# alexfreudenberg/miraculix

Hardware: AMD Instinct MI355X
Metric: effective GFLOP/s for dgemm_compressed (2-bit SNP x fp64) (higher is better)
Workload: dtype f64; 1 GPU; 1000000x50000 (SNPs x indiv), ncol=32, dgemm_compressed N+T per step, uncentred; snps=1000000, indiv=50000, ncol=32, parallelism=snp-shard1, form=one process per GPU

## Files before the change

miraculix_amd/csrc/mxa_api.cpp:

```cpp
#include "../../include/miraculix_amd.h"
#include "mxa_internal.h"

#include <algorithm>
#include <atomic>
#include <chrono>
#include <cstdarg>
#include <cstdio>
#include <cstdlib>
#include <cstring>
#include <mutex>
#include <string>
#include <vector>

namespace mxa {

static int g_err = 0;
static char g_errmsg[512] = "";

Options &options() { static Options o; return o; }
Profile &profile() { static Profile p; return p; }
Geometry &last_geometry() { static Geometry g; return g; }
static bool g_profile_on = true;
static std::atomic<int> g_engine{[] {
  const char *e = getenv("MXA_ENGINE");
// ... 585 lines not shown
  const PackedMatrix *G_tn_single = no_plain ? &gemm_operand(h, trans, true) : nullptr;
  const bool small_ok = (engine == 0 || (engine == 4 && n <= 2)) && k >= 128;
  auto guarded_small = [&](int c0, int nc, const PackedMatrix *G_tn, hipEvent_t e0, hipEvent_t e1, int *splits_out, const int **flag_ptr) -> int {
    I8Chain ch; ch.S0 = kSmallS0[nc]; ch.S1 = kSmallS1[nc];
    const bool fb_lut = nc <= 2 && !no_plain;
    GemmPlan pf = fb_lut ? plan_lut(m, G.k_pad, nc) : plan_gemm(m, G.k_pad, nc);
    bool fast_fb = nc >= 2;
    if (fast_fb) {
      const size_t one = (size_t)pf.n_pad * pf.m_pad, need = one * pf.splits;
      fast_fb = partial_budget(w, need, one) >= need;
    }
    ch.fp64_rows = !fast_fb;
    const int r0 = gemm_i8_reserve(G, nc, ch.S0, G_tn, w, s);
    if (r0) return r0;
    if (ch.S1) {
      const int r1 = gemm_i8_reserve(G, nc, ch.S1, G_tn, w, s);
      if (r1 == 1) return 1;
      if (r1 == 2) ch.S1 = 0;
    }
    const double *dBc = dB + (size_t)c0 * ldb;
    double *dCc = dC + (size_t)c0 * ldc;
    const int *d_flag = nullptr;
    for (int cls = 0; cls < (ch.S1 ? 2 : 1); cls++) {
      ch.my_class = cls; ch.first = cls == 0;
      const int rc = gemm_i8_device(G, trans, nc, dBc, ldb, dCc, ldc, fill_rows, centered, d_sumB + c0, d_sumfB + c0, h->d_f, w, s, cls == 0 ? e0 : nullptr, cls == 0 ? e1 : nullptr,
                                    cls == 0 ? splits_out : nullptr, 2, &d_flag, w.d_colpart, 0, G_tn, nullptr, &ch);
      if (rc != 3) return 1;
    }
    if (fast_fb) {
      if (ensure_partials(w, pf, s)) return 1;
      if (fb_lut) { if (launch_lut(G, dBc, ldb, nc, w.d_P, pf, s, d_flag)) return 1; }
      else {
        const bool trf = gemm_use_tr(pf, h, trans);
        if (launch_pack_B(dBc, ldb, k, nc, w.d_Bp, G.k_pad, pf.n_pad, pf.c, s, nullptr, 0, -1, d_flag)) return 1;
        if (launch_gemm(gemm_operand(h, trans, trf), w.d_Bp, w.d_P, pf, 0, s, next_ctr(w), 0, -1, d_flag, trf)) return 1;
      }
      if (launch_finish(w.d_P, pf, m, nc, dCc, ldc, fill_rows, trans ? 1 : 0, centered, d_sumB + c0, d_sumfB + c0, h->d_f, s, nullptr, 0, 0, d_flag, nullptr)) return 1;
    }
    if (flag_ptr) *flag_ptr = d_flag;
    return 0;
  };
  if (small_ok && n <= kSmallNMaxColsHost) {
    const char *e_tn = getenv("MXA_I8_TN");
    const bool tn_ab = e_tn && atoi(e_tn) != 0;
    const PackedMatrix *G_tn = no_plain ? G_tn_single : (tn_ab && n <= 2 && !h->single) ? &gemm_operand(h, trans, true) : nullptr;
    int splits8 = 1;
    const int *d_flag = nullptr;
    const int rcx = guarded_small(0, n, G_tn, pe0, pe1, &splits8, &d_flag);
    if (rcx == 1) return 1;
    if (rcx == 0) {
      std::lock_guard<std::mutex> lk(g_prof_mutex);
      Geometry &geo = last_geometry();
      geo.m = m; geo.k = k; geo.n = n; geo.splits = splits8; geo.a = 0; geo.c = 0; geo.path = 4; geo.d_flag = d_flag; geo.flag_dev = h->device;
      h->prof_pending[slot] = prof;
      return 0;
    }
  }
  if (centered && launch_colsums(dB, ldb, k, n, trans ? nullptr : h->d_f, w.d_colpart, d_sumB, d_sumfB, s)) return 1;
  auto i8_engine_product = [&](int S, double *stats_base, hipEvent_t e0, hipEvent_t e1, int *splits_out) -> int {
    const int rc = gemm_i8_device(G, trans, n, dB, ldb, dC, ldc, fill_rows, centered, d_sumB, d_sumfB, h->d_f, w, s, e0, e1, splits_out, 0, nullptr, nullptr, S, G_tn_single, stats_base);
    if (rc != 2 || !G_tn_single) return rc;
    const int cmax = (6 * 32) / (S > 0 ? S : 7);
    if (cmax < 1) return 2;
    const int chunks = (n + cmax - 1) / cmax, per = (n + chunks - 1) / chunks;
    if (chunks < 2) return 2;
    for (int c0 = 0; c0 < n; c0 += per) {
      const int nc = std::min(per, n - c0);
      const int rcc = gemm_i8_device(G, trans, nc, dB + (size_t)c0 * ldb, ldb, dC + (size_t)c0 * ldc, ldc, fill_rows, centered, d_sumB + c0, d_sumfB + c0, h->d_f, w, s,
// ... 42 lines not shown
  const bool use_lut = n <= 2 && !no_plain;
  GemmPlan p = use_lut ? plan_lut(m, G.k_pad, n) : plan_gemm(m, G.k_pad, n);
  int splits_per_group = p.splits;
  if (!use_lut) {
    const size_t one = (size_t)p.n_pad * p.m_pad, need = one * p.splits;
    const size_t budget = partial_budget(w, need, one);
    if (budget < need) {
      splits_per_group = (int)std::max<size_t>(1, budget / one);
      GemmPlan pg = p; pg.splits = splits_per_group;
      if (ensure_partials(w, pg, s)) return 1;
    }
  }
  if (splits_per_group == p.splits && ensure_partials(w, p, s)) return 1;
  clock_mark("partials");
  {
    std::lock_guard<std::mutex> lk(g_prof_mutex);
    Geometry &geo = last_geometry();
    geo.m = m; geo.k = k; geo.n = n; geo.splits = p.splits; geo.a = p.a; geo.c = p.c; geo.path = use_lut ? 1 : 0;
  }
  const bool tr = !use_lut && gemm_use_tr(p, h, trans);
  const PackedMatrix &GL = gemm_operand(h, trans, tr);
  int mode = gemm_default_mode(p.c);
  const int *d_E = nullptr;
  if (!use_lut && (mode == 2 || mode == 3)) {
    if (w.cap_exp < (size_t)n) {
      MXA_HIP(hipStreamSynchronize(s));
      if (w.d_exp) { MXA_HIP(hipFree(w.d_exp)); w.d_exp = nullptr; w.cap_exp = 0; }
      MXA_HIP(hipMalloc(reinterpret_cast<void **>(&w.d_exp), sizeof(int) * (size_t)n));
      w.cap_exp = n;
    }
    if (launch_colexp(dB, ldb, k, n, w.d_colpart, w.d_exp, 0, s, w.d_denflag, kDenMaxSpan, -100000)) return 1;
    d_E = w.d_exp;
  }
  if (!use_lut && launch_pack_B(dB, ldb, k, n, w.d_Bp, G.k_pad, p.n_pad, p.c, s, d_E, 0, -1, nullptr, mode == 3 && !tr)) return 1;
  if (prof) MXA_HIP(hipEventRecord(pe0, s));
  if (splits_per_group < p.splits) {
    const size_t stride = (size_t)p.n_pad * p.m_pad;
    for (int pass = 0; pass < (d_E ? 2 : 1); pass++) {
      const int *gate = pass ? w.d_denflag : nullptr;
      if (pass && launch_pack_B(dB, ldb, k, n, w.d_Bp, G.k_pad, p.n_pad, p.c, s, nullptr, 0, -1, gate)) return 1;
      for (int sb = 0; sb < p.splits; sb += splits_per_group) {
        const int se = std::min(p.splits, sb + splits_per_group);
        if ((size_t)(se - sb) * stride > w.cap_P) { set_error(4, "internal: a group of %d K splits exceeds the partial-sum workspace", se - sb); return 1; }
        if (launch_gemm(GL, w.d_Bp, w.d_P, p, pass ? 0 : mode, s, next_ctr(w), sb, se, gate, tr, sb)) return 1;
        const int group = (sb > 0 ? 1 : 0) | (se < p.splits ? 2 : 0);
        if (launch_finish(w.d_P, p, m, n, dC, ldc, fill_rows, trans ? 1 : 0, centered, d_sumB, d_sumfB, h->d_f, s, pass ? nullptr : d_E, 0, 0, gate, nullptr, se - sb, group)) return 1;
      }
      if (!pass && prof) { MXA_HIP(hipEventRecord(pe1, s)); h->prof_pending[slot] = true; }
    }
    return 0;
  }
  int rc = use_lut ? launch_lut(G, dB, ldb, n, w.d_P, p, s) : launch_gemm(GL, w.d_Bp, w.d_P, p, mode, s, next_ctr(w), 0, -1, nullptr, tr);
  if (prof && !rc) { MXA_HIP(hipEventRecord(pe1, s)); h->prof_pending[slot] = true; }
  if (!rc && d_E) {
    rc = launch_pack_B(dB, ldb, k, n, w.d_Bp, G.k_pad, p.n_pad, p.c, s, nullptr, 0, -1, w.d_denflag);
    if (!rc) rc = launch_gemm(GL, w.d_Bp, w.d_P, p, 0, s, next_ctr(w), 0, -1, w.d_denflag, tr);
  }
  if (!rc) rc = launch_finish(w.d_P, p, m, n, dC, ldc, fill_rows, trans ? 1 : 0, centered, d_sumB, d_sumfB, h->d_f, s, d_E, 0, 0, nullptr, d_E ? w.d_denflag : nullptr);
  return rc;
}


constexpr int kPipeChunks = 8;
static const size_t kPipeMinBytes = (size_t)32 << 20;

static int pipe_setup(Handle *h) {
  for (hipStream_t &ps : h->pipe) if (!ps) MXA_HIP(hipStreamCreateWithFlags(&ps, hipStreamNonBlocking));
  for (hipEvent_t &e : h->pev) if (!e) MXA_HIP(hipEventCreateWithFlags(&e, hipEventDisableTiming));
  return 0;
}

static int gemm_host_pipelined(Handle *h, bool trans, int n, const double *B, long ldb, bool b_host, bool b_local, double *C, long ldc, bool c_host, bool c_local,
                               long fill_rows) {
  const int engine = g_engine.load();
  if ((engine != 0 && engine != 3) || n < 3 || getenv("MXA_DIAG")) return 2;
  if (engine == 0 && n <= kSmallNMaxColsHost) return 2;
  const PackedMatrix &G = trans ? h->snp_major : h->ind_major;
  const long m = G.rows, k = G.k;
  const size_t b_bytes = b_host ? sizeof(double) * (size_t)k * n : 0, c_bytes = c_host ? sizeof(double) * (size_t)m * n : 0;
  if (std::max(b_bytes, c_bytes) < kPipeMinBytes) return 2;
  const bool kmode = b_bytes >= c_bytes;
  const bool centered = options().centered;
  if (centered && !h->has_f) { set_error(6, "dgemm_compressed: centring requested but no allele frequencies were supplied to plink2compressed"); return 1; }
  if (n > h->max_n) h->max_n = n;
  if (ensure_workspace(h, n) || pipe_setup(h)) return 1;
  harvest_profile(h);
  Workspace &w = h->ws;
  hipStream_t s = h->stream;
  if (grow(&w.d_colpart, &w.cap_colpart, (size_t)n * (128 * (kPipeChunks + 1) + 2) + 16)) return 1;
// ... 765 lines not shown
```

miraculix_amd/csrc/mxa_internal.h:

```cpp
#pragma once
#include <hip/hip_runtime.h>
#include <cstddef>
#include <cstdint>
#include <functional>
#include <utility>
#include <vector>
#include "mxa_plan.h"

namespace mxa {

constexpr int kWaves = 4;
constexpr int kKStep = 16;
constexpr int kSlabSteps = 8;
constexpr int kSlabK = kKStep * kSlabSteps;
constexpr int kSlabBytes = kSlabK / 4;
constexpr int kRowAlign = 512;
constexpr int kTileRows = 256;
constexpr int kTileBytes = kTileRows * kSlabBytes;

constexpr long kMaxBlocksPerLaunch = 1L << 23;
template <typename Launch>
inline void launch_in_block_chunks(long blocks, Launch &&launch) {
  for (long b0 = 0; b0 < blocks; b0 += kMaxBlocksPerLaunch) launch((unsigned)(blocks - b0 < kMaxBlocksPerLaunch ? blocks - b0 : kMaxBlocksPerLaunch), b0);
}
// ... 106 lines not shown
int bed_range_to_handle(const char *base, long snps_total, long indiv, long snp_begin, long snp_end, int max_n, int device, void **out,
                        double *f_out_local);
constexpr int kMaxShards = 64;
struct PartList { const double *p[kMaxShards]; int count; };
int launch_reduce_parts(const PartList &parts, long m, int n, double *dC, long ldc, long fill_rows, hipStream_t s);

void set_error(int code, const char *fmt, ...);
void clear_error();
bool check_hip(hipError_t e, const char *func, int line);
#define MXA_HIP(x) do { if (!::mxa::check_hip((x), __func__, __LINE__)) return 1; } while (0)
void debug_info(const char *fmt, ...);
struct CallClock {
  bool on = false;
  double t0 = 0.0, last = 0.0;
  char line[512]; int len = 0;
  static double now();
  void start(bool enabled) { on = enabled; len = 0; line[0] = 0; if (on) t0 = last = now(); }
  void mark(const char *what);
  void report(const char *head);
};
extern thread_local CallClock *tl_call_clock;
inline void clock_mark(const char *what) { if (tl_call_clock && tl_call_clock->on) tl_call_clock->mark(what); }

int launch_recode(const uint8_t *d_src, size_t src_pitch, long row0, long nrows, long k, long k_bit_offset,
                  PackedMatrix &dst, hipStream_t s);
constexpr int kDenUp = 900;
constexpr int kDenMaxSpan = 800;
constexpr int kI8ExactMaxDigits = 24;
int launch_colspan(const double *dB, long ldb, long k, int n, double *d_part, int *d_out3, hipStream_t s);
int launch_colexp_from_part(const double *d_part, int n, int *d_E, int bias, hipStream_t s);
int launch_colexp(const double *dB, long ldb, long k, int n, double *d_part, int *d_E, int bias, hipStream_t s, int *d_flag = nullptr, int max_span = 0,
                  int min_emax = 0, bool reset_flag = true);
int launch_pack_B(const double *dB, long ldb, long k, int n, double *dBp, long k_pad, int n_pad, int c, hipStream_t s, const int *d_E = nullptr, long S0 = 0,
                  long S_cnt = -1, const int *run_if_set = nullptr, bool rowscale = false);
int launch_colsums(const double *dB, long ldb, long k, int n, const double *d_f , double *d_part,
                   double *d_sumB, double *d_sumfB, hipStream_t s);
GemmPlan plan_gemm(long m, long k_pad, int n, const GemmPlan *ksplits_like = nullptr);
int gemm_default_mode(int c);
int launch_gemm(const PackedMatrix &G, const double *dBp, double *dP, const GemmPlan &p, int mode, hipStream_t s, int *d_ctr, int split_begin = 0, int split_end = -1,
                const int *run_if_set = nullptr, bool tr = false, int p_split0 = 0);
GemmPlan plan_lut(long m, long k_pad, int n);
int launch_lut(const PackedMatrix &G, const double *dB, long ldb, int n, double *dP, const GemmPlan &p, hipStream_t s, const int *run_if_set = nullptr);
int launch_finish(const double *dP, const GemmPlan &p, long m, int n, double *dC, long ldc, long fill_rows, int mode_trans,
                  bool centered, const double *d_sumB, const double *d_sumfB, const double *d_f, hipStream_t s, const int *d_E = nullptr, int e_splits = 0,
                  int e_stride = 0, const int *run_if_set = nullptr, const int *unscaled_if_set = nullptr, int group_splits = 0, int group = 0);
int ensure_dyn_lds(const void *func, int bytes, unsigned long long *mask);
int launch_transpose_2bit(const uint8_t *d_in, long rows, long cols, uint8_t *d_out, hipStream_t s);
int launch_allele_freq(const uint8_t *d_plink, long snps, long indiv, double *d_f, hipStream_t s);
int launch_plink_lut(uint8_t *d, size_t nbytes, hipStream_t s);
int launch_sparse_times_plink(const uint8_t *dP, size_t pitch, long entries, int nIdx, const int *d_rowIdx, const int *d_colIdx, const double *d_val,
                              double *dC_slab, long ldc, long e_base, long e_count, hipStream_t s);
struct I8Chain { int S0 = 0, S1 = 0, my_class = 0; bool first = true; bool fp64_rows = true; };
int gemm_i8_device(const PackedMatrix &G, bool trans, int n, const double *dB, long ldb, double *dC, long ldc, long fill_rows, bool centered, double *d_sumB,
                   double *d_sumfB, const double *d_f, Workspace &w, hipStream_t s, hipEvent_t ev0, hipEvent_t ev1, int *splits_out, int guard = 0,
                   const int **flag_out = nullptr, double *colsum_scratch = nullptr, int S_override = 0, const PackedMatrix *G_tn = nullptr,
                   double *stats_part = nullptr, const I8Chain *chain = nullptr);
int gemm_i8_reserve(const PackedMatrix &G, int n, int S, const PackedMatrix *G_tn, Workspace &w, hipStream_t s);

int ld_window_any(const char *who, const unsigned char *plink, long snps, long indiv, long window, const int *last, double *out, long ldb, bool scores, int flag,
                  bool is_plink, const double *freq);
int ld_pairwise_any(const char *who, const unsigned char *plink, long snps, long indiv, long window, const int *last, double *out, long ldb, bool scores, int flag);

int launch_dgemm(bool ta, bool tb, long M, long N, long K, double alpha, const double *A, long lda, const double *B, long ldb, double beta, double *C, long ldc,
                 bool lower_only, hipStream_t s);
int launch_potrf_inv_block(double *A, long ld, int nb, long offset, int *info, double *inv_out, hipStream_t s);

}
```

miraculix_amd/csrc/mxa_kernels.hip:

```cpp
#include "mxa_internal.h"
#include "mxa_queue.h"
#include <algorithm>
#include <cstdio>
#include <cstdlib>
#include <vector>

namespace mxa {


__device__ __forceinline__ uint32_t recode16(uint32_t w) {
  const uint32_t H = (w >> 1) & 0x55555555u, L = w & 0x55555555u;
  return ((H & L) << 1) | (H & ~L);
}

__global__ void __launch_bounds__(256) k_recode(const uint8_t *__restrict__ src, size_t src_pitch, long src_row_bytes,
                                                long nrows, long k, uint8_t *__restrict__ dst, long dst_row0, long nslabs, long rows_blocks, long blk0) {
  const long bid = blk0 + blockIdx.x;
  const long rblk = bid % rows_blocks, sgrp = bid / rows_blocks;
  const int rr = threadIdx.x >> 3, part = threadIdx.x & 7;
  const long r = rblk * 32 + rr;
  const long slab = sgrp * 4 + (part >> 1);
  if (r >= nrows || slab >= nslabs) return;
  const long b = slab * kSlabBytes + (part & 1) * 16;
  uint32_t w[4] = {0u, 0u, 0u, 0u};
  const uint8_t *p = src + (size_t)r * src_pitch + b;
  if (b + 16 <= src_row_bytes && (reinterpret_cast<size_t>(p) & 3) == 0) {
    const uint32_t *q = reinterpret_cast<const uint32_t *>(p);
    w[0] = q[0]; w[1] = q[1]; w[2] = q[2]; w[3] = q[3];
  } else {
    for (int u = 0; u < 16; u++)
      if (b + u < src_row_bytes) w[u >> 2] |= (uint32_t)p[u] << (8 * (u & 3));
  }
#pragma unroll
  for (int i = 0; i < 4; i++) {
    uint32_t x = recode16(w[i]);
    const long valid = k - 4 * (b + 4 * i);
    if (valid <= 0) x = 0;
    else if (valid < 16) x &= (1u << (2 * valid)) - 1u;
    w[i] = x;
  }
  const long R = dst_row0 + r;
  const size_t off = ((size_t)(R / kTileRows) * nslabs + (size_t)slab) * kTileBytes + (size_t)(R % kTileRows) * kSlabBytes + (part & 1) * 16;
  *reinterpret_cast<uint4 *>(dst + off) = make_uint4(w[0], w[1], w[2], w[3]);
}

int launch_recode(const uint8_t *d_src, size_t src_pitch, long row0, long nrows, long k, long ,
                  PackedMatrix &dst, hipStream_t s) {
  if (nrows <= 0) return 0;
  const long rows_blocks = (nrows + 31) / 32, slab_groups = (dst.nslabs + 3) / 4;
  const long grid = rows_blocks * slab_groups;
  for (long b0 = 0; b0 < grid; b0 += kMaxBlocksPerLaunch) {
    const long nb = std::min(kMaxBlocksPerLaunch, grid - b0);
    hipLaunchKernelGGL(k_recode, dim3((unsigned)nb), dim3(256), 0, s, d_src, src_pitch, (k + 3) / 4, nrows, k, dst.d, row0, dst.nslabs, rows_blocks, b0);
  }
  MXA_HIP(hipGetLastError());
  return 0;
}

__host__ __device__ __forceinline__ long gemm_k_index(long S, int kk) { return (S >> 3) * 128 + 16 * (kk & 7) + 8 * (kk >> 3) + (S & 7); }

__global__ void __launch_bounds__(256) k_pack_B(const double *__restrict__ B, long ldb, long k, int n,
                                                double *__restrict__ Bp, long total, int C, long S_total, const int *__restrict__ E, int up, long S0, long S_cnt,
                                                const int *__restrict__ run_if_set, int rowscale) {
  if (run_if_set && *run_if_set == 0) return;
  for (long idx = (long)blockIdx.x * blockDim.x + threadIdx.x; idx < total; idx += (long)gridDim.x * blockDim.x) {
    const int l = (int)(idx & 63);
    const long sh = idx >> 6;
    const int h = (int)(sh % C);
    const long cs = sh / C;
    const long S = S0 + cs % S_cnt;
    const int chunk = (int)(cs / S_cnt);
    const long row = gemm_k_index(S, l >> 2);
    const int col = chunk * 4 * C + 4 * h + (l & 3);
    double v = 0.0;
    if (row < k && col < n) {
      v = B[row + (long)col * ldb];
      if (E) v = ldexp(v, up - E[col] - (rowscale ? 2 * (int)(row & 15) : 0));
    }
    Bp[(((size_t)chunk * S_total + S) * C + h) * 64 + l] = v;
  }
}

__global__ void __launch_bounds__(256) k_colmax_partial(const double *__restrict__ B, long ldb, long k, double *__restrict__ part, int n, int want_min) {
  const int j = blockIdx.y, c = blockIdx.x;
  const long per = (k + 63) / 64;
  const long c0 = c * per, c1 = std::min<long>(k, c0 + per);
  const double inf = __longlong_as_double(0x7ff0000000000000ll);
  double m = 0.0, lo = inf;
  for (long r = c0 + threadIdx.x; r < c1; r += 256) {
    const double a = fabs(B[r + (long)j * ldb]);
    m = (a <= 1.7976931348623157e308) ? fmax(m, a) : inf;
    if (a > 0.0) lo = fmin(lo, a);
  }
  __shared__ double sh[256], sl[256];
  sh[threadIdx.x] = m; sl[threadIdx.x] = lo;
  __syncthreads();
// ... 41 lines not shown
  __shared__ int s_span[256], s_emax[256], s_bad[256];
  int span = 0, emin_max = 1 << 20, bad = 0;
  for (int j = threadIdx.x; j < n; j += 256) {
    double m = 0.0;
    for (int c = 0; c < 64; c++) m = fmax(m, part[(size_t)j * 64 + c]);
    if (!isfinite(m)) { bad = 1; continue; }
    if (m > 0.0) {
      double lo = m;
      for (int c = 0; c < 64; c++) lo = fmin(lo, part[((size_t)n + j) * 64 + c]);
      int e = 0, el = 0;
      (void)frexp(m, &e); (void)frexp(lo, &el);
      span = max(span, e - el); emin_max = min(emin_max, e);
    }
  }
  s_span[threadIdx.x] = span; s_emax[threadIdx.x] = emin_max; s_bad[threadIdx.x] = bad;
  __syncthreads();
  for (int w = 128; w > 0; w >>= 1) {
    if ((int)threadIdx.x < w) {
      s_span[threadIdx.x] = max(s_span[threadIdx.x], s_span[threadIdx.x + w]); s_emax[threadIdx.x] = min(s_emax[threadIdx.x], s_emax[threadIdx.x + w]);
      s_bad[threadIdx.x] |= s_bad[threadIdx.x + w];
    }
    __syncthreads();
  }
  if (threadIdx.x == 0) { out[0] = s_span[0]; out[1] = s_emax[0] == (1 << 20) ? 0 : s_emax[0]; out[2] = s_bad[0]; }
}
int launch_colspan(const double *dB, long ldb, long k, int n, double *d_part, int *d_out3, hipStream_t s) {
  hipLaunchKernelGGL(k_colmax_partial, dim3(64, n), dim3(256), 0, s, dB, ldb, k, d_part, n, 1);
  hipLaunchKernelGGL(k_colspan_final, dim3(1), dim3(256), 0, s, d_part, n, d_out3);
  MXA_HIP(hipGetLastError());
  return 0;
}

int launch_pack_B(const double *dB, long ldb, long k, int n, double *dBp, long k_pad, int n_pad, int c, hipStream_t s, const int *d_E, long S0, long S_cnt,
                  const int *run_if_set, bool rowscale) {
  const long S_total = k_pad / 16;
  if (S_cnt < 0) S_cnt = S_total - S0;
  const long total = S_cnt * (long)(n_pad / 4) * 64;
  if (total <= 0) return 0;
  const int grid = (int)std::min<long>((total + 255) / 256, 256L * 64);
  hipLaunchKernelGGL(k_pack_B, dim3(grid), dim3(256), 0, s, dB, ldb, k, n, dBp, total, c, S_total, d_E, kDenUp, S0, S_cnt, run_if_set, rowscale ? 1 : 0);
  MXA_HIP(hipGetLastError());
  return 0;
}

constexpr int kColChunks = 64;

__global__ void __launch_bounds__(256) k_colsum_partial(const double *__restrict__ B, long ldb, long k,
                                                        const double *__restrict__ f, double *__restrict__ part) {
  const int j = blockIdx.y, c = blockIdx.x;
  const long per = (k + kColChunks - 1) / kColChunks;
  const long c0 = c * per, c1 = std::min<long>(k, c0 + per);
  double s1 = 0.0, s2 = 0.0;
  for (long r = c0 + threadIdx.x; r < c1; r += 256) {
    const double b = B[r + (long)j * ldb];
    s1 += b;
    if (f) s2 = fma(f[r], b, s2);
  }
  __shared__ double sh1[256], sh2[256];
  sh1[threadIdx.x] = s1; sh2[threadIdx.x] = s2;
  __syncthreads();
  for (int w = 128; w > 0; w >>= 1) {
    if ((int)threadIdx.x < w) { sh1[threadIdx.x] += sh1[threadIdx.x + w]; sh2[threadIdx.x] += sh2[threadIdx.x + w]; }
    __syncthreads();
  }
  if (threadIdx.x == 0) {
    part[((size_t)j * kColChunks + c) * 2 + 0] = sh1[0];
    part[((size_t)j * kColChunks + c) * 2 + 1] = sh2[0];
  }
}

__global__ void k_colsum_final(const double *__restrict__ part, int n, double *__restrict__ sumB, double *__restrict__ sumfB) {
  const int j = blockIdx.x * blockDim.x + threadIdx.x;
  if (j >= n) return;
// ... 260 lines not shown
              Pbase[(size_t)col * Cfg::kRowsWG + row] = out;
            }
          }
        }
      }
      asm volatile("s_waitcnt lgkmcnt(0)" ::: "memory");
      __builtin_amdgcn_wave_barrier();
    }
    if (DIAG && threadIdx.x == 0 && diag) {
      diag[2 * (size_t)bid] = t1 - t0; diag[2 * (size_t)bid + 1] = r1 - r0;
      diag[2 * (size_t)nunits + 2 * (size_t)bid] = rt_begin; diag[2 * (size_t)nunits + 2 * (size_t)bid + 1] = r0;
      diag[4 * (size_t)nunits + bid] = __builtin_amdgcn_s_memrealtime();
    }
    if (next < 0) break;
    u = un; bid = next;
    asm volatile("s_waitcnt vmcnt(0)" ::: "memory");
    __syncthreads();
  }
}

int gemm_default_mode(int) {
  return 3;
}

static long device_cus() {
  static const long r = [] {
    int dev = 0; hipDeviceProp_t prop;
    if (hipGetDevice(&dev) != hipSuccess || hipGetDeviceProperties(&prop, dev) != hipSuccess) { (void)hipGetLastError(); return 256L; }
    return (long)prop.multiProcessorCount;
  }();
  return r > 0 ? r : 256;
}

GemmPlan plan_gemm(long m, long k_pad, int n, const GemmPlan *ksplits_like) { return plan_gemm_host(m, k_pad, n, device_cus(), ksplits_like); }

template <int A, int C, int MODE, bool TR = false>
static int launch_gemm_t(const PackedMatrix &G, const double *dBp, double *dP, const GemmPlan &p, hipStream_t s, int split_begin, int split_end, const int *run_if_set,
                         int *d_ctr, int p_split0) {
  using Cfg = GemmCfg<A, C>;
  static unsigned long long attr_mask = 0;
  if (ensure_dyn_lds(reinterpret_cast<const void *>(&k_gemm<A, C, MODE, false, TR>), Cfg::kLds, &attr_mask)) return 1;
  const long nunits = (long)p.rowblocks * p.nchunks * (split_end - split_begin);
  if (nunits > 0x3fffffffL) { set_error(3, "launch too large"); return 1; }
  if (nunits <= 0) return 0;
  if (!d_ctr) { set_error(4, "internal: k_gemm needs its queue counters"); return 1; }
  static int per_cu[64] = {};
  int dev = 0;
  MXA_HIP(hipGetDevice(&dev));
  if (!per_cu[dev & 63]) {
    int nb = 0;
    MXA_HIP(hipOccupancyMaxActiveBlocksPerMultiprocessor(&nb, reinterpret_cast<const void *>(&k_gemm<A, C, MODE, false, TR>), 256, Cfg::kLds));
    hipDeviceProp_t prop;
    MXA_HIP(hipGetDeviceProperties(&prop, dev));
    per_cu[dev & 63] = std::max(1, std::min(nb, gemm_wg_per_cu(C))) * prop.multiProcessorCount;
  }
  const long grid = std::min<long>(nunits, per_cu[dev & 63]);
  constexpr int xcd_order = 1;
  const KSplit ks{p.s1, p.l1, p.r1, p.l2};
  const int long_groups = (std::min(split_end, p.s1) - std::min(split_begin, p.s1)) * p.nchunks;
  const int g8 = xcd_order ? (long_groups & ~7) : 0;
  MXA_HIP(hipMemsetAsync(d_ctr, 0, 9 * sizeof(int), s));
  static const bool diag_on = getenv("MXA_DIAG") != nullptr;
  if (!TR && diag_on && ((A == 8 && C == 8) || (A == 16 && C == 1)) && split_begin == 0 && split_end == p.splits && !run_if_set) {
    static unsigned long long attr2 = 0;
    if (ensure_dyn_lds(reinterpret_cast<const void *>(&k_gemm<A, C, MODE, true>), Cfg::kLds, &attr2)) return 1;
    unsigned long long *d_diag = nullptr;
    MXA_HIP(hipMalloc(reinterpret_cast<void **>(&d_diag), sizeof(unsigned long long) * 5 * nunits));
    MXA_HIP(hipMemsetAsync(d_diag, 0, sizeof(unsigned long long) * 5 * nunits, s));
    hipLaunchKernelGGL((k_gemm<A, C, MODE, true>), dim3((unsigned)grid), dim3(256), Cfg::kLds, s, G.d, G.pitch, dBp, p.n_pad / 4, dP,
                       p.m_pad, p.n_pad, p.rowblocks, p.nchunks, p.slabs_total, ks, xcd_order, d_diag, split_begin, (const int *)nullptr, (int)nunits, d_ctr, g8, p_split0);
    MXA_HIP(hipStreamSynchronize(s));
    std::vector<unsigned long long> h(5 * nunits);
    MXA_HIP(hipMemcpy(h.data(), d_diag, sizeof(unsigned long long) * 5 * nunits, hipMemcpyDeviceToHost));
    std::vector<double> ghz, cyc;
    for (long i = 0; i < nunits; i++) if (h[2 * i + 1]) {
      const int sp = (int)(i < (long)g8 * p.rowblocks ? ((i & 7) + 8 * ((i >> 3) / p.rowblocks)) / p.nchunks : (i / p.rowblocks) / p.nchunks);
      const int len = ksplit_len(ks, sp);
      ghz.push_back((double)h[2 * i] / (double)h[2 * i + 1] * 0.1); cyc.push_back((double)h[2 * i] / len);
    }
    std::sort(ghz.begin(), ghz.end()); std::sort(cyc.begin(), cyc.end());
    if (!ghz.empty()) printf("MXA_DIAG k_gemm<%d,%d,%d>: %ld pieces on %ld workgroups (splits %d = %d x %d + short x %d), in-kernel clock median %.3f GHz (min %.3f max %.3f); shader cycles per slab median %.0f (ideal %d)\n",
                             A, C, MODE, nunits, grid, p.splits, p.s1, p.l1, p.l2, ghz[ghz.size() / 2], ghz.front(), ghz.back(), cyc[cyc.size() / 2], kSlabSteps * A * C * 16 * 2);
    double ticks = 0.0;
    for (long i = 0; i < nunits; i++) ticks += (double)h[2 * i + 1];
    printf("MXA_DIAG k_gemm: K loops of all pieces = %.3f ms if packed perfectly on %ld resident slots (compare with the kernel duration)\n", ticks * 1e-5 / (double)grid, grid);
    {
      double life = 0; unsigned long long first = ~0ull, last = 0;
      for (long i = 0; i < nunits; i++) {
        const unsigned long long b = h[2 * nunits + 2 * i], e = h[4 * nunits + i];
        life += (double)(e - b);
        first = std::min(first, b); last = std::max(last, e);
      }
      printf("MXA_DIAG k_gemm: mean piece lifetime %.1f us; span first begin -> last end %.3f ms; sum of lifetimes / slots = %.3f ms\n",
             life / nunits * 1e-2, (double)(last - first) * 1e-5, life * 1e-5 / (double)grid);
      std::vector<std::pair<unsigned long long, int>> ev;
      ev.reserve(2 * nunits);
      for (long i = 0; i < nunits; i++) { ev.emplace_back(h[2 * nunits + 2 * i], +1); ev.emplace_back(h[4 * nunits + i], -1); }
      std::sort(ev.begin(), ev.end());
      const unsigned long long win = 200000;
      double idle[3] = {0, 0, 0}; long active = 0, max_active = 0; unsigned long long prev_t = first;
      for (auto &e : ev) {
        unsigned long long t0 = prev_t, t1 = e.first;
        while (t0 < t1) {
          const int zone = t0 < first + win ? 0 : (t0 >= last - win ? 2 : 1);
          const unsigned long long border = zone == 0 ? first + win : (zone == 1 ? last - win : last);
          const unsigned long long te = std::min(t1, std::max(border, t0 + 1));
          idle[zone] += (double)(te - t0) * (double)(grid - std::min(active, grid));
          t0 = te;
        }
        active += e.second; max_active = std::max(max_active, active); prev_t = e.first;
      }
      printf("MXA_DIAG k_gemm: idle slot-time first 2 ms %.3f ms, middle %.3f ms, last 2 ms %.3f ms; max pieces in flight %ld\n",
             idle[0] * 1e-5 / (double)grid, idle[1] * 1e-5 / (double)grid, idle[2] * 1e-5 / (double)grid, max_active);
    }
    (void)hipFree(d_diag);
    return 0;
  }
  hipLaunchKernelGGL((k_gemm<A, C, MODE, false, TR>), dim3((unsigned)grid), dim3(256), Cfg::kLds, s, G.d, G.pitch, dBp, p.n_pad / 4, dP,
                     p.m_pad, p.n_pad, p.rowblocks, p.nchunks, p.slabs_total, ks, xcd_order, (unsigned long long *)nullptr, split_begin, run_if_set, (int)nunits, d_ctr, g8, p_split0);
  MXA_HIP(hipGetLastError());
  return 0;
}

int launch_gemm(const PackedMatrix &G, const double *dBp, double *dP, const GemmPlan &p, int mode, hipStream_t s, int *d_ctr, int split_begin, int split_end,
                const int *run_if_set, bool tr, int p_split0) {
  if (split_end < 0) split_end = p.splits;
  if (p_split0 < 0 || p_split0 > split_begin) { set_error(4, "internal: k_gemm partial-sum base split %d outside [0, %d]", p_split0, split_begin); return 1; }
  if (!G.d) { set_error(4, "internal: k_gemm was given a packed matrix that is not stored (single-orientation object)"); return 1; }
  if (tr) {
    if ((long)p.slabs_total * kSlabK > G.rows_pad || G.nslabs < 1 || (mode != 0 && mode != 3)) {
      set_error(4, "internal: transposed launch does not fit the packed matrix (K slabs %d x 128 > %ld rows) or mode %d", p.slabs_total, G.rows_pad, mode);
      return 1;
    }
#define MXA_DISPATCH_TR(AA, CC)                                                                                          \
    if (p.a == AA && p.c == CC) {                                                                                        \
      if (mode == 3) return launch_gemm_t<AA, CC, 3, true>(G, dBp, dP, p, s, split_begin, split_end, nullptr, d_ctr, p_split0);     \
      return launch_gemm_t<AA, CC, 0, true>(G, dBp, dP, p, s, split_begin, split_end, run_if_set, d_ctr, p_split0);                 \
    }
    MXA_DISPATCH_TR(16, 1) MXA_DISPATCH_TR(16, 2) MXA_DISPATCH_TR(16, 3) MXA_DISPATCH_TR(16, 4)
    MXA_DISPATCH_TR(8, 5) MXA_DISPATCH_TR(8, 6) MXA_DISPATCH_TR(8, 7) MXA_DISPATCH_TR(8, 8)
#undef MXA_DISPATCH_TR
    set_error(5, "internal: no transposed kernel for tile a=%d c=%d", p.a, p.c);
    return 1;
  }
  if (p.m_pad > G.rows_pad || (size_t)p.slabs_total * kSlabBytes > G.pitch) {
    set_error(4, "internal: packed matrix smaller than the launch plan (m_pad %ld > %ld or k bytes %ld > pitch %zu)", p.m_pad,
              G.rows_pad, (long)p.slabs_total * kSlabBytes, G.pitch);
    return 1;
  }
#define MXA_DISPATCH(AA, CC)                                              \
  if (p.a == AA && p.c == CC) {                                           \
    if (mode == 3) return launch_gemm_t<AA, CC, 3>(G, dBp, dP, p, s, split_begin, split_end, nullptr, d_ctr, p_split0);     \
    return launch_gemm_t<AA, CC, 0>(G, dBp, dP, p, s, split_begin, split_end, run_if_set, d_ctr, p_split0);                 \
  }
  MXA_DISPATCH(16, 1)
  MXA_DISPATCH(16, 2)
  MXA_DISPATCH(16, 3)
  MXA_DISPATCH(16, 4)
  MXA_DISPATCH(8, 5)
  MXA_DISPATCH(8, 6)
  MXA_DISPATCH(8, 7)
  MXA_DISPATCH(8, 8)
#undef MXA_DISPATCH
  set_error(5, "internal: no kernel for tile a=%d c=%d", p.a, p.c);
  return 1;
}

template <int NV, int KS, int WV>
struct LutCfg {
  static constexpr int kThreads = 64 * WV;
  static constexpr int kRows = kThreads;
  static constexpr int kChunks = KS / 64;
  static constexpr int kRowBytes = kRows * KS / 4;
  static constexpr int kTabBytes = (KS / 2) * 16 * 8 * NV;
  static constexpr int kBufBytes = kRowBytes + kTabBytes;
  static constexpr int kLds = 2 * kBufBytes;
};

template <int NV, int KS, int WV>
__global__ void __launch_bounds__(64 * WV)
k_lut(const uint8_t *__restrict__ G, size_t pitch, const double *__restrict__ B, long ldb, long k, int n, double *__restrict__ P,
      long m_pad, int rowblocks, int slabs_total, int slabs_per_split, const int *__restrict__ run_if_set) {
  using Cfg = LutCfg<NV, KS, WV>;
  extern __shared__ __attribute__((aligned(16))) char smem[];
  if (run_if_set && *run_if_set == 0) return;
  const int tid = threadIdx.x, lane = tid & 63;
// ... 401 lines not shown
```

miraculix_amd/csrc/mxa_plan.h:

```cpp
#pragma once
#include <algorithm>
#include <cstddef>
#include <vector>

#if defined(__HIPCC__)
#define MXA_HD __host__ __device__
#else
#define MXA_HD
#endif

namespace mxa {

constexpr int kPlanWaves = 4;
constexpr int kPlanSlabSteps = 8;
constexpr int kPlanSlabK = 128;
constexpr int kPlanLutWaves = 8;
constexpr int kPlanLutKS = 128;

struct KSplit { int s1, l1, r1, l2; };
MXA_HD inline int ksplit_begin(const KSplit &ks, int sp) {
  return sp < ks.s1 ? sp * ks.l1 + (sp < ks.r1 ? sp : ks.r1) : ks.s1 * ks.l1 + ks.r1 + (sp - ks.s1) * ks.l2;
}
MXA_HD inline int ksplit_len(const KSplit &ks, int sp) { return sp < ks.s1 ? ks.l1 + (sp < ks.r1 ? 1 : 0) : ks.l2; }
inline int ksplit_make(KSplit &ks, long total, long l1_target, long lt, long tail_units) {
  long s2 = 0;
  if (lt > 0 && tail_units > 0 && 2 * lt <= l1_target) s2 = (tail_units + lt - 1) / lt;
  while (s2 > 0 && s2 * lt > total / 2) s2--;
  const long longpart = total - s2 * lt;
  long s1 = longpart > 0 ? (longpart + l1_target - 1) / l1_target : 0;
  if (s1 < 1 && longpart > 0) s1 = 1;
  const long l1 = s1 ? longpart / s1 : 0;
  ks.s1 = (int)s1; ks.l1 = (int)l1; ks.r1 = (int)(s1 ? longpart - s1 * l1 : 0); ks.l2 = (int)(s2 ? lt : l1);
  return (int)(s1 + s2);
}


struct GemmPlan { int a, c, nchunks, n_pad, splits, slabs_per_split, slabs_total, rowblocks; long m_pad; long p_rows; int s1, l1, l2, r1; };
inline long plan_split_begin(const GemmPlan &p, int sp) {
  return sp < p.s1 ? (long)sp * p.l1 + (sp < p.r1 ? sp : p.r1) : (long)p.s1 * p.l1 + p.r1 + (long)(sp - p.s1) * p.l2;
}

inline int gemm_wg_per_cu(int c) { return c == 1 ? 4 : c == 2 ? 3 : 2; }

inline GemmPlan plan_gemm_host(long m, long k_pad, int n, long cus, const GemmPlan *ksplits_like = nullptr) {
  GemmPlan p{};
  p.nchunks = (n + 31) / 32;
  const int per = (n + p.nchunks - 1) / p.nchunks;
  p.c = (per + 3) / 4;
  p.a = p.c <= 4 ? 16 : 8;
  const int cols_chunk = 4 * p.c;
  p.n_pad = p.nchunks * cols_chunk;
  const int rows_wg = kPlanWaves * 4 * p.a;
  p.rowblocks = (int)((m + rows_wg - 1) / rows_wg);
  p.m_pad = (long)p.rowblocks * rows_wg;
  p.p_rows = rows_wg;
  p.slabs_total = (int)(k_pad / kPlanSlabK);
  if (ksplits_like) {
    p.splits = ksplits_like->splits; p.s1 = ksplits_like->s1; p.l1 = ksplits_like->l1; p.l2 = ksplits_like->l2; p.r1 = ksplits_like->r1; p.slabs_per_split = ksplits_like->slabs_per_split;
    return p;
  }
  constexpr double piece_us = 1500.0, tail_us = 200.0;
  const long units = (long)p.rowblocks * p.nchunks;
  const long resident = gemm_wg_per_cu(p.c) * cus;
  const double slab_us = (double)kPlanSlabSteps * p.a * p.c * 16.0 * gemm_wg_per_cu(p.c) / 2390.0;
  long l1 = std::max<long>(8, std::min<long>(p.slabs_total, (long)(piece_us / slab_us + 0.5)));
  constexpr long b_l2_bytes = 3L << 20;
  {
    const long cap = b_l2_bytes / ((long)p.c * 4096);
    l1 = std::max<long>(8, std::min<long>(l1, cap));
  }
  while (l1 > 16 && units * ((p.slabs_total + l1 - 1) / l1) < 6 * resident) l1 = l1 * 3 / 4;
  const long lt = tail_us > 0 ? std::max<long>(8, (long)(tail_us / slab_us + 0.5)) : 0;
  const bool taper = lt > 0 && units * ((p.slabs_total + l1 - 1) / l1) >= 3 * resident;
  const long tail = taper ? lt * std::max<long>(1, (5 * resident / 2 + units - 1) / units) : 0;
  KSplit ks;
  p.splits = ksplit_make(ks, p.slabs_total, l1, lt, tail);
  p.s1 = ks.s1; p.l1 = ks.l1; p.r1 = ks.r1; p.l2 = ks.l2;
  l1 = ks.l1;
  p.slabs_per_split = (int)l1;
  if (p.splits < 1) p.splits = 1;
  return p;
}


inline GemmPlan plan_lut_host(long m, long k_pad, int n) {
  GemmPlan p{};
  p.a = 0; p.c = 0;
  p.n_pad = n <= 1 ? 1 : n <= 2 ? 2 : 4;
  p.nchunks = 1;
  p.rowblocks = (int)((m + 64 * kPlanLutWaves - 1) / (64 * kPlanLutWaves));
  p.m_pad = (long)p.rowblocks * 64 * kPlanLutWaves;
  p.p_rows = p.m_pad;
  p.slabs_total = (int)(k_pad / kPlanLutKS);
  const long units = p.rowblocks;
  constexpr long target = 8192L;
  long want = (target + units - 1) / units;
  long max_splits = std::max<long>(1, p.slabs_total / 16);
  long splits = std::max<long>(1, std::min<long>(want, max_splits));
  p.slabs_per_split = (int)((p.slabs_total + splits - 1) / splits);
  p.splits = (p.slabs_total + p.slabs_per_split - 1) / p.slabs_per_split;
  p.s1 = p.splits; p.l1 = p.l2 = p.slabs_per_split; p.r1 = 0;
  return p;
}


constexpr int kTnPieceCost = 20;
constexpr int kTnMaxPieces = 64;
constexpr int kTnMaxPieceStages = 2047;
constexpr long kTnTailWindowBytes = 3L << 20;
constexpr int kTnTailMinStages = 96;
struct TnSched { int mode, strips, K, slots, pslots, q0, q1, q2; };
struct TnItem { int strip, st0, stages, slot; };
MXA_HD inline int tn_tail_begin(int Q, int nb, int b) { return (int)((unsigned)b * (unsigned)Q / (unsigned)nb); }
MXA_HD inline int tn_tail_owner(int Q, int nb, int g) { return (int)((((unsigned)g + 1u) * (unsigned)nb - 1u) / (unsigned)Q); }
// ... 106 lines not shown
```

Measured before the change: 74420 GFLOP/s.

## Choose GEMM K-split plan via scheduling simulation; fold counter reset into pack kernel

Adds a host-side model that simulates how work units are dispatched across XCD queues, and uses it to search alternative K-split lengths and tail configurations. The search picks a plan only if it lowers the modelled makespan plus finish cost, and plans are memoized per shape. Separately, the work-queue counter is zeroed inside the pack_B kernel instead of a separate hipMemsetAsync before each GEMM launch, removing one stream operation. The risks are added host planning cost on first call and plans that are tuned to a model that may not match the hardware.

```diff
diff --git a/miraculix_amd/csrc/mxa_api.cpp b/miraculix_amd/csrc/mxa_api.cpp
--- a/miraculix_amd/csrc/mxa_api.cpp
+++ b/miraculix_amd/csrc/mxa_api.cpp
@@ -641,8 +641,9 @@
       if (fb_lut) { if (launch_lut(G, dBc, ldb, nc, w.d_P, pf, s, d_flag)) return 1; }
       else {
         const bool trf = gemm_use_tr(pf, h, trans);
-        if (launch_pack_B(dBc, ldb, k, nc, w.d_Bp, G.k_pad, pf.n_pad, pf.c, s, nullptr, 0, -1, d_flag)) return 1;
-        if (launch_gemm(gemm_operand(h, trans, trf), w.d_Bp, w.d_P, pf, 0, s, next_ctr(w), 0, -1, d_flag, trf)) return 1;
+        int *ctr = next_ctr(w);
+        if (launch_pack_B(dBc, ldb, k, nc, w.d_Bp, G.k_pad, pf.n_pad, pf.c, s, nullptr, 0, -1, d_flag, false, ctr)) return 1;
+        if (launch_gemm(gemm_operand(h, trans, trf), w.d_Bp, w.d_P, pf, 0, s, ctr, 0, -1, d_flag, trf, 0, true)) return 1;
       }
       if (launch_finish(w.d_P, pf, m, nc, dCc, ldc, fill_rows, trans ? 1 : 0, centered, d_sumB + c0, d_sumfB + c0, h->d_f, s, nullptr, 0, 0, d_flag, nullptr)) return 1;
     }
@@ -751,7 +752,9 @@
     if (launch_colexp(dB, ldb, k, n, w.d_colpart, w.d_exp, 0, s, w.d_denflag, kDenMaxSpan, -100000)) return 1;
     d_E = w.d_exp;
   }
-  if (!use_lut && launch_pack_B(dB, ldb, k, n, w.d_Bp, G.k_pad, p.n_pad, p.c, s, d_E, 0, -1, nullptr, mode == 3 && !tr)) return 1;
+  const bool one_launch = !use_lut && splits_per_group == p.splits;
+  int *ctr = one_launch ? next_ctr(w) : nullptr;
+  if (!use_lut && launch_pack_B(dB, ldb, k, n, w.d_Bp, G.k_pad, p.n_pad, p.c, s, d_E, 0, -1, nullptr, mode == 3 && !tr, ctr)) return 1;
   if (prof) MXA_HIP(hipEventRecord(pe0, s));
   if (splits_per_group < p.splits) {
     const size_t stride = (size_t)p.n_pad * p.m_pad;
@@ -769,11 +772,12 @@
     }
     return 0;
   }
-  int rc = use_lut ? launch_lut(G, dB, ldb, n, w.d_P, p, s) : launch_gemm(GL, w.d_Bp, w.d_P, p, mode, s, next_ctr(w), 0, -1, nullptr, tr);
+  int rc = use_lut ? launch_lut(G, dB, ldb, n, w.d_P, p, s) : launch_gemm(GL, w.d_Bp, w.d_P, p, mode, s, ctr, 0, -1, nullptr, tr, 0, true);
   if (prof && !rc) { MXA_HIP(hipEventRecord(pe1, s)); h->prof_pending[slot] = true; }
   if (!rc && d_E) {
-    rc = launch_pack_B(dB, ldb, k, n, w.d_Bp, G.k_pad, p.n_pad, p.c, s, nullptr, 0, -1, w.d_denflag);
-    if (!rc) rc = launch_gemm(GL, w.d_Bp, w.d_P, p, 0, s, next_ctr(w), 0, -1, w.d_denflag, tr);
+    int *ctr_fb = next_ctr(w);
+    rc = launch_pack_B(dB, ldb, k, n, w.d_Bp, G.k_pad, p.n_pad, p.c, s, nullptr, 0, -1, w.d_denflag, false, ctr_fb);
+    if (!rc) rc = launch_gemm(GL, w.d_Bp, w.d_P, p, 0, s, ctr_fb, 0, -1, w.d_denflag, tr, 0, true);
   }
   if (!rc) rc = launch_finish(w.d_P, p, m, n, dC, ldc, fill_rows, trans ? 1 : 0, centered, d_sumB, d_sumfB, h->d_f, s, d_E, 0, 0, nullptr, d_E ? w.d_denflag : nullptr);
   return rc;
diff --git a/miraculix_amd/csrc/mxa_internal.h b/miraculix_amd/csrc/mxa_internal.h
--- a/miraculix_amd/csrc/mxa_internal.h
+++ b/miraculix_amd/csrc/mxa_internal.h
@@ -162,13 +162,13 @@
 int launch_colexp(const double *dB, long ldb, long k, int n, double *d_part, int *d_E, int bias, hipStream_t s, int *d_flag = nullptr, int max_span = 0,
                   int min_emax = 0, bool reset_flag = true);
 int launch_pack_B(const double *dB, long ldb, long k, int n, double *dBp, long k_pad, int n_pad, int c, hipStream_t s, const int *d_E = nullptr, long S0 = 0,
-                  long S_cnt = -1, const int *run_if_set = nullptr, bool rowscale = false);
+                  long S_cnt = -1, const int *run_if_set = nullptr, bool rowscale = false, int *zero_ctr = nullptr);
 int launch_colsums(const double *dB, long ldb, long k, int n, const double *d_f , double *d_part,
                    double *d_sumB, double *d_sumfB, hipStream_t s);
 GemmPlan plan_gemm(long m, long k_pad, int n, const GemmPlan *ksplits_like = nullptr);
 int gemm_default_mode(int c);
 int launch_gemm(const PackedMatrix &G, const double *dBp, double *dP, const GemmPlan &p, int mode, hipStream_t s, int *d_ctr, int split_begin = 0, int split_end = -1,
-                const int *run_if_set = nullptr, bool tr = false, int p_split0 = 0);
+                const int *run_if_set = nullptr, bool tr = false, int p_split0 = 0, bool ctr_zeroed = false);
 GemmPlan plan_lut(long m, long k_pad, int n);
 int launch_lut(const PackedMatrix &G, const double *dB, long ldb, int n, double *dP, const GemmPlan &p, hipStream_t s, const int *run_if_set = nullptr);
 int launch_finish(const double *dP, const GemmPlan &p, long m, int n, double *dC, long ldc, long fill_rows, int mode_trans,
diff --git a/miraculix_amd/csrc/mxa_kernels.hip b/miraculix_amd/csrc/mxa_kernels.hip
--- a/miraculix_amd/csrc/mxa_kernels.hip
+++ b/miraculix_amd/csrc/mxa_kernels.hip
@@ -3,6 +3,10 @@
 #include <algorithm>
 #include <cstdio>
 #include <cstdlib>
+#include <map>
+#include <mutex>
+#include <string>
+#include <tuple>
 #include <vector>
 
 namespace mxa {
@@ -61,7 +65,8 @@
 
 __global__ void __launch_bounds__(256) k_pack_B(const double *__restrict__ B, long ldb, long k, int n,
                                                 double *__restrict__ Bp, long total, int C, long S_total, const int *__restrict__ E, int up, long S0, long S_cnt,
-                                                const int *__restrict__ run_if_set, int rowscale) {
+                                                const int *__restrict__ run_if_set, int rowscale, int *__restrict__ zero_ctr) {
+  if (zero_ctr && blockIdx.x == 0 && threadIdx.x < 9) zero_ctr[threadIdx.x] = 0;
   if (run_if_set && *run_if_set == 0) return;
   for (long idx = (long)blockIdx.x * blockDim.x + threadIdx.x; idx < total; idx += (long)gridDim.x * blockDim.x) {
     const int l = (int)(idx & 63);
@@ -169,13 +174,16 @@
 }
 
 int launch_pack_B(const double *dB, long ldb, long k, int n, double *dBp, long k_pad, int n_pad, int c, hipStream_t s, const int *d_E, long S0, long S_cnt,
-                  const int *run_if_set, bool rowscale) {
+                  const int *run_if_set, bool rowscale, int *zero_ctr) {
   const long S_total = k_pad / 16;
   if (S_cnt < 0) S_cnt = S_total - S0;
   const long total = S_cnt * (long)(n_pad / 4) * 64;
-  if (total <= 0) return 0;
+  if (total <= 0) {
+    if (zero_ctr) MXA_HIP(hipMemsetAsync(zero_ctr, 0, 9 * sizeof(int), s));
+    return 0;
+  }
   const int grid = (int)std::min<long>((total + 255) / 256, 256L * 64);
-  hipLaunchKernelGGL(k_pack_B, dim3(grid), dim3(256), 0, s, dB, ldb, k, n, dBp, total, c, S_total, d_E, kDenUp, S0, S_cnt, run_if_set, rowscale ? 1 : 0);
+  hipLaunchKernelGGL(k_pack_B, dim3(grid), dim3(256), 0, s, dB, ldb, k, n, dBp, total, c, S_total, d_E, kDenUp, S0, S_cnt, run_if_set, rowscale ? 1 : 0, zero_ctr);
   MXA_HIP(hipGetLastError());
   return 0;
 }
@@ -502,11 +510,25 @@
   return r > 0 ? r : 256;
 }
 
-GemmPlan plan_gemm(long m, long k_pad, int n, const GemmPlan *ksplits_like) { return plan_gemm_host(m, k_pad, n, device_cus(), ksplits_like); }
+GemmPlan plan_gemm(long m, long k_pad, int n, const GemmPlan *ksplits_like) {
+  const long cus = device_cus();
+  if (ksplits_like) return plan_gemm_host(m, k_pad, n, cus, ksplits_like);
+  const char *knob = getenv("MXA_GEMM_PLAN");
+  static std::mutex mu;
+  static std::map<std::tuple<long, long, int, long, std::string>, GemmPlan> memo;
+  const auto key = std::make_tuple(m, k_pad, n, cus, std::string(knob ? knob : ""));
+  std::lock_guard<std::mutex> lk(mu);
+  const auto it = memo.find(key);
+  if (it != memo.end()) return it->second;
+  const GemmPlan p = plan_gemm_host(m, k_pad, n, cus, nullptr, knob);
+  if (memo.size() >= 4096) memo.clear();
+  memo.emplace(key, p);
+  return p;
+}
 
 template <int A, int C, int MODE, bool TR = false>
 static int launch_gemm_t(const PackedMatrix &G, const double *dBp, double *dP, const GemmPlan &p, hipStream_t s, int split_begin, int split_end, const int *run_if_set,
-                         int *d_ctr, int p_split0) {
+                         int *d_ctr, int p_split0, bool ctr_zeroed) {
   using Cfg = GemmCfg<A, C>;
   static unsigned long long attr_mask = 0;
   if (ensure_dyn_lds(reinterpret_cast<const void *>(&k_gemm<A, C, MODE, false, TR>), Cfg::kLds, &attr_mask)) return 1;
@@ -529,7 +551,7 @@
   const KSplit ks{p.s1, p.l1, p.r1, p.l2};
   const int long_groups = (std::min(split_end, p.s1) - std::min(split_begin, p.s1)) * p.nchunks;
   const int g8 = xcd_order ? (long_groups & ~7) : 0;
-  MXA_HIP(hipMemsetAsync(d_ctr, 0, 9 * sizeof(int), s));
+  if (!ctr_zeroed) MXA_HIP(hipMemsetAsync(d_ctr, 0, 9 * sizeof(int), s));
   static const bool diag_on = getenv("MXA_DIAG") != nullptr;
   if (!TR && diag_on && ((A == 8 && C == 8) || (A == 16 && C == 1)) && split_begin == 0 && split_end == p.splits && !run_if_set) {
     static unsigned long long attr2 = 0;
@@ -593,7 +615,7 @@
 }
 
 int launch_gemm(const PackedMatrix &G, const double *dBp, double *dP, const GemmPlan &p, int mode, hipStream_t s, int *d_ctr, int split_begin, int split_end,
-                const int *run_if_set, bool tr, int p_split0) {
+                const int *run_if_set, bool tr, int p_split0, bool ctr_zeroed) {
   if (split_end < 0) split_end = p.splits;
   if (p_split0 < 0 || p_split0 > split_begin) { set_error(4, "internal: k_gemm partial-sum base split %d outside [0, %d]", p_split0, split_begin); return 1; }
   if (!G.d) { set_error(4, "internal: k_gemm was given a packed matrix that is not stored (single-orientation object)"); return 1; }
@@ -604,8 +626,8 @@
     }
 #define MXA_DISPATCH_TR(AA, CC)                                                                                          \
     if (p.a == AA && p.c == CC) {                                                                                        \
-      if (mode == 3) return launch_gemm_t<AA, CC, 3, true>(G, dBp, dP, p, s, split_begin, split_end, nullptr, d_ctr, p_split0);     \
-      return launch_gemm_t<AA, CC, 0, true>(G, dBp, dP, p, s, split_begin, split_end, run_if_set, d_ctr, p_split0);                 \
+      if (mode == 3) return launch_gemm_t<AA, CC, 3, true>(G, dBp, dP, p, s, split_begin, split_end, nullptr, d_ctr, p_split0, ctr_zeroed);     \
+      return launch_gemm_t<AA, CC, 0, true>(G, dBp, dP, p, s, split_begin, split_end, run_if_set, d_ctr, p_split0, ctr_zeroed);                 \
     }
     MXA_DISPATCH_TR(16, 1) MXA_DISPATCH_TR(16, 2) MXA_DISPATCH_TR(16, 3) MXA_DISPATCH_TR(16, 4)
     MXA_DISPATCH_TR(8, 5) MXA_DISPATCH_TR(8, 6) MXA_DISPATCH_TR(8, 7) MXA_DISPATCH_TR(8, 8)
@@ -620,8 +642,8 @@
   }
 #define MXA_DISPATCH(AA, CC)                                              \
   if (p.a == AA && p.c == CC) {                                           \
-    if (mode == 3) return launch_gemm_t<AA, CC, 3>(G, dBp, dP, p, s, split_begin, split_end, nullptr, d_ctr, p_split0);     \
-    return launch_gemm_t<AA, CC, 0>(G, dBp, dP, p, s, split_begin, split_end, run_if_set, d_ctr, p_split0);                 \
+    if (mode == 3) return launch_gemm_t<AA, CC, 3>(G, dBp, dP, p, s, split_begin, split_end, nullptr, d_ctr, p_split0, ctr_zeroed);     \
+    return launch_gemm_t<AA, CC, 0>(G, dBp, dP, p, s, split_begin, split_end, run_if_set, d_ctr, p_split0, ctr_zeroed);                 \
   }
   MXA_DISPATCH(16, 1)
   MXA_DISPATCH(16, 2)
diff --git a/miraculix_amd/csrc/mxa_plan.h b/miraculix_amd/csrc/mxa_plan.h
--- a/miraculix_amd/csrc/mxa_plan.h
+++ b/miraculix_amd/csrc/mxa_plan.h
@@ -1,6 +1,8 @@
 #pragma once
 #include <algorithm>
 #include <cstddef>
+#include <cstdlib>
+#include <utility>
 #include <vector>
 
 #if defined(__HIPCC__)
@@ -42,7 +44,10 @@
 
 inline int gemm_wg_per_cu(int c) { return c == 1 ? 4 : c == 2 ? 3 : 2; }
 
-inline GemmPlan plan_gemm_host(long m, long k_pad, int n, long cus, const GemmPlan *ksplits_like = nullptr) {
+inline long gemm_l1_cap(int c) { return (3L << 20) / ((long)c * 4096); }
+inline double gemm_slab_us_nominal(int a, int c) { return (double)kPlanSlabSteps * a * c * 16.0 * gemm_wg_per_cu(c) / 2390.0; }
+
+inline GemmPlan plan_gemm_host_v1(long m, long k_pad, int n, long cus, const GemmPlan *ksplits_like = nullptr) {
   GemmPlan p{};
   p.nchunks = (n + 31) / 32;
   const int per = (n + p.nchunks - 1) / p.nchunks;
@@ -80,6 +85,133 @@
   p.slabs_per_split = (int)l1;
   if (p.splits < 1) p.splits = 1;
   return p;
+}
+
+inline double gemm_sim_launch(const KSplit &ks, int splits, long rowblocks, int nchunks, long resident, double slab_us, double piece_fixed_us,
+                              std::vector<unsigned char> *executed = nullptr) {
+  const long groups = (long)nchunks * splits, nunits = groups * rowblocks;
+  if (nunits <= 0 || resident <= 0) return 0.0;
+  const long g8 = ((long)std::min(splits, ks.s1) * nchunks) & ~7L;
+  const long qsize[9] = {(g8 / 8) * rowblocks, (g8 / 8) * rowblocks, (g8 / 8) * rowblocks, (g8 / 8) * rowblocks, (g8 / 8) * rowblocks, (g8 / 8) * rowblocks,
+                         (g8 / 8) * rowblocks, (g8 / 8) * rowblocks, nunits - g8 * rowblocks};
+  if (executed) executed->assign((size_t)nunits, 0);
+  const long long slab_ns = (long long)(slab_us * 1000.0 + 0.5), fixed_ns = (long long)(piece_fixed_us * 1000.0 + 0.5);
+  const long grid = std::min(nunits, resident);
+  long head[9] = {0, 0, 0, 0, 0, 0, 0, 0, 0}, run_end[9] = {0, 0, 0, 0, 0, 0, 0, 0, 0};
+  auto group_len = [&](int q, long gi) { return ksplit_len(ks, (int)((q < 8 ? q + 8 * gi : g8 + gi) / nchunks)); };
+  std::vector<std::pair<long long, long>> free_at[8];
+  for (int x = 0; x < 8; x++) { const long c = grid / 8 + (x < grid % 8 ? 1 : 0); if (c > 0) free_at[x].emplace_back(0LL, c); }
+  long long makespan = 0;
+  for (;;) {
+    int bx = -1; long long bt = 0;
+    for (int x = 0; x < 8; x++) if (!free_at[x].empty() && (bx < 0 || free_at[x].front().first < bt)) { bx = x; bt = free_at[x].front().first; }
+    if (bx < 0) break;
+    std::vector<std::pair<long long, long>> &F = free_at[bx];
+    int q = -1;
+    for (int phase = 0; phase <= 8 && q < 0; phase++) { const int y = phase == 0 ? bx : phase == 1 ? 8 : ((bx + phase - 1) & 7); if (head[y] < qsize[y]) q = y; }
+    if (q < 0) { makespan = std::max(makespan, bt); F.erase(F.begin()); continue; }
+    const long gi = head[q] / rowblocks;
+    const int len = group_len(q, gi);
+    if (run_end[q] <= head[q]) {
+      long ge = gi + 1;
+      const long gq = qsize[q] / rowblocks;
+      while (ge < gq && group_len(q, ge) == len) ge++;
+      run_end[q] = ge * rowblocks;
+    }
+    const long take = std::min(F.front().second, run_end[q] - head[q]);
+    if (executed) for (long i = head[q]; i < head[q] + take; i++) { unsigned char &e = (*executed)[(size_t)(q < 8 ? i * 8 + q : g8 * rowblocks + i)]; if (e < 255) e++; }
+    head[q] += take;
+    if (F.front().second == take) F.erase(F.begin()); else F.front().second -= take;
+    const long long t1 = bt + (long long)len * slab_ns + fixed_ns;
+    auto it = std::lower_bound(F.begin(), F.end(), std::make_pair(t1, 0L));
+    if (it != F.end() && it->first == t1) it->second += take; else F.insert(it, std::make_pair(t1, take));
+  }
+  return (double)makespan * 1e-3;
+}
+
+constexpr double kModelPieceFixedUs = 9.0;
+constexpr double kModelSlabScale = 1.027;
+constexpr double kModelFinishGBs = 5500.0;
+constexpr double kModelMaxLaunchUs = 20000.0;
+constexpr double kModelMinLaunchUs = 1000.0;
+constexpr long kModelMaxPieces = 1L << 16;
+constexpr double kModelMinGain = 0.01;
+constexpr bool kModelDefaultOn = true;
+
+inline double gemm_plan_model_us(const GemmPlan &p, long cus, double *launch_us = nullptr) {
+  const KSplit ks{p.s1, p.l1, p.r1, p.l2};
+  const double launch = gemm_sim_launch(ks, p.splits, p.rowblocks, p.nchunks, gemm_wg_per_cu(p.c) * cus, gemm_slab_us_nominal(p.a, p.c) * kModelSlabScale, kModelPieceFixedUs);
+  if (launch_us) *launch_us = launch;
+  return launch + (double)p.splits * (double)p.n_pad * (double)p.m_pad * 8.0 / (kModelFinishGBs * 1e3);
+}
+
+inline GemmPlan plan_gemm_host_forced(long m, long k_pad, int n, long cus, long l1, long l2, long short_splits) {
+  GemmPlan p = plan_gemm_host_v1(m, k_pad, n, cus);
+  const long total = p.slabs_total;
+  l1 = std::max<long>(1, std::min<long>(l1, std::max<long>(1, total)));
+  l2 = std::max<long>(0, std::min<long>(l2, total));
+  short_splits = std::max<long>(0, std::min<long>(short_splits, total));
+  KSplit ks;
+  p.splits = ksplit_make(ks, total, l1, l2, short_splits * l2);
+  p.s1 = ks.s1; p.l1 = ks.l1; p.r1 = ks.r1; p.l2 = ks.l2;
+  p.slabs_per_split = ks.l1;
+  if (p.splits < 1) p.splits = 1;
+  return p;
+}
+
+inline GemmPlan plan_gemm_host_model(long m, long k_pad, int n, long cus) {
+  const GemmPlan v1 = plan_gemm_host_v1(m, k_pad, n, cus);
+  const long resident = gemm_wg_per_cu(v1.c) * cus;
+  const double slab_us = gemm_slab_us_nominal(v1.a, v1.c) * kModelSlabScale;
+  const double ideal = (double)v1.rowblocks * v1.nchunks * (double)v1.slabs_total * slab_us / (double)resident;
+  if (ideal > kModelMaxLaunchUs || ideal < kModelMinLaunchUs || v1.slabs_total < 16 || (long)v1.rowblocks * v1.nchunks * v1.splits > kModelMaxPieces) return v1;
+  double launch_v1 = 0.0;
+  const double cost_v1 = gemm_plan_model_us(v1, cus, &launch_v1);
+  GemmPlan best = v1; double best_cost = cost_v1;
+  auto consider = [&](long l1, long l2, long s2) {
+    if (l1 < 16 || l1 > std::max<long>(gemm_l1_cap(v1.c), v1.l1 + 1)) return;
+    const GemmPlan c = plan_gemm_host_forced(m, k_pad, n, cus, l1, l2, s2);
+    const long pieces = (long)c.rowblocks * c.nchunks * c.splits;
+    if (pieces > kModelMaxPieces || pieces < std::min<long>((long)v1.rowblocks * v1.nchunks * v1.splits, 6 * resident)) return;
+    if (((long)c.s1 * c.nchunks) % 8 > ((long)v1.s1 * v1.nchunks) % 8) return;
+    double launch = 0.0;
+    const double cost = gemm_plan_model_us(c, cus, &launch);
+    if (cost < best_cost && launch <= launch_v1) { best = c; best_cost = cost; }
+  };
+  const long l1_v1 = v1.l1 + (v1.r1 ? 1 : 0), s2_v1 = v1.splits - v1.s1;
+  if (s2_v1 == 0) return v1;
+  const long l2s[] = {8, 16, 22, v1.l2};
+  const long l1s[] = {l1_v1, std::min<long>(gemm_l1_cap(v1.c), v1.slabs_total), l1_v1 * 3 / 4};
+  for (long l1 : l1s) {
+    consider(l1, 0, 0);
+    for (long l2 : l2s)
+      for (long s2 = 1; s2 <= s2_v1 && l2 <= v1.l2; s2++) consider(l1, l2, s2);
+  }
+  return best_cost <= cost_v1 * (1.0 - kModelMinGain) ? best : v1;
+}
+
+inline GemmPlan plan_gemm_host_knob(long m, long k_pad, int n, long cus, const char *knob) {
+  if (knob && *knob) {
+    long v[3] = {0, 0, 0}; int cnt = 0;
+    const char *s = knob;
+    while (cnt < 3) {
+      char *end = nullptr;
+      const long x = strtol(s, &end, 10);
+      if (end == s) break;
+      v[cnt++] = x;
+      if (*end != ',') { s = end; break; }
+      s = end + 1;
+    }
+    if (cnt == 3 && *s == 0) return plan_gemm_host_forced(m, k_pad, n, cus, v[0], v[1], v[2]);
+    if (cnt == 1 && *s == 0 && v[0] == 0) return plan_gemm_host_v1(m, k_pad, n, cus);
+    if (cnt == 1 && *s == 0 && v[0] == 1) return plan_gemm_host_model(m, k_pad, n, cus);
+  }
+  return kModelDefaultOn ? plan_gemm_host_model(m, k_pad, n, cus) : plan_gemm_host_v1(m, k_pad, n, cus);
+}
+
+inline GemmPlan plan_gemm_host(long m, long k_pad, int n, long cus, const GemmPlan *ksplits_like = nullptr, const char *knob = nullptr) {
+  if (ksplits_like) return plan_gemm_host_v1(m, k_pad, n, cus, ksplits_like);
+  return plan_gemm_host_knob(m, k_pad, n, cus, knob);
 }
 
 
```

New measurement: 74350 GFLOP/s, median of 2. No clear change (-0.1%).
